# zoj613/OccuSpytial

Hardware: AMD Instinct MI355X
Metric: Gibbs iterations/sec on 100x100 ICAR lattice, 4 chains; 1/2/4/8 GPUs (higher is better)
Workload: dtype f64; 1 GPU; 100x100 queen ICAR lattice, 10000 sites, 5 visits/site, p=q=2, 4 chains per GPU batched in every kernel (BASELINE configs[1] data, the metric's 4 chains); chains_per_gpu=4, total_chains=4, sites=10000, visit_rows=50000, parallelism=chains sharded 4/GPU, no data-path collective; one GPU, communicator=single process, problem_transport=none, krylov_cap=0, stalls=0, solve_form=k_iter, one XCD per chain, solve_workgroups_per_chain=23, main_stream_cus=160, fused_fallbacks=0, threads_per_block=64

## Files before the change

### occuspytial_amd/csrc/occ_gibbs.hip

```cpp
#include "../../include/occ_gibbs.h"

#include <hip/hip_runtime.h>
#include <hip/hip_ext.h>

#include <algorithm>
#include <chrono>
#include <cmath>
#include <cstdio>
#include <cstdlib>
#include <cstring>
#include <atomic>
#include <map>
#include <mutex>
#include <string>
#include <thread>
#include <vector>

#include "occ_comm.hpp"
#include "occ_tiles.hpp"
#include "occ_comp.hpp"
#include "occ_rsr.hpp"
#include "occ_probit.hpp"
#include "occ_spatial.hpp"
#include "occ_hist.hpp"
// ... 109 lines not shown
        CompArgs args{};
        std::vector<void *> dev;
    } comp;
    bool comp_on() const { return comp.args.k > 1; }
    struct Switches {
        uint32_t any = 0u;
        std::vector<uint32_t> on;
        uint32_t *on_dev = nullptr;
    };
    struct Spatial : Switches {
        SpArgs args{};
    } spatial;
    struct AccumRun : Switches {
        bool ready = false, snapped = false;
        uint8_t *data = nullptr, *count = nullptr, *snap = nullptr;
        size_t unit = 0;
    };
    struct Hist : AccumRun {
        std::vector<uint64_t> bound;
        HistArgs args{};
    } hist;
    struct Conv : AccumRun {
        ConvArgs args{};
    } conv;
    struct Holdout : AccumRun {
        std::vector<double> packed;
        HoldoutArgs args{};
    } holdout;
    AccumRun &accum(int kind) { return kind == ACC_HIST ? (AccumRun &)hist : kind == ACC_CONV ? (AccumRun &)conv : (AccumRun &)holdout; }
    std::vector<ChainScalars> snap_sc;
    std::vector<std::pair<void *, size_t>> fixed_list;
    std::vector<const char *> fixed_names;
    bool defer_fixed = false;
    std::string group_transport = "none";
    Inject *inj_dev = nullptr;
    double *inj_u = nullptr;
    int snap_parity = 0;
    int64_t fused_fallbacks = 0;
    bool streams_serialised = false;
    unsigned *probe_w = nullptr;
    unsigned long long probe_gen = 0;
    int64_t stream_probes = 0, repromotions = 0;
    unsigned *sync_buf = nullptr;
    bool demoted = false;
    int promote_wait = 0, promote_backoff = 1;
    std::string pair_note;
    std::vector<ChainScalars> mirror;
    bool mirror_ok = false;
    bool clean_exit = false;
    ChainScalars *pin_sc = nullptr;
    double *pin_rec = nullptr;
    size_t pin_rec_cap = 0;
    bool marks_done = false;
    bool debug_close_window = false;
    bool wedged = false;
    int probe_wait = 0, probe_backoff = 1;
    int graph_parity = 0;
    std::vector<void *> allocs;
    std::string err;
    int launch_rc = 0;
    std::string launch_err;
    int parity = 0;
    bool need_prologue = true;
    hipGraph_t head_graph[2] = {nullptr, nullptr}, tail_graph[2] = {nullptr, nullptr};
    hipGraphExec_t head[2] = {nullptr, nullptr}, tail[2] = {nullptr, nullptr};
    hipEvent_t ev_z[2] = {nullptr, nullptr}, ev_side[2] = {nullptr, nullptr};
    int krylov_cap = 0;
    int64_t iterations = 0, graph_launches = 0, eager_iterations = 0, stalls = 0;
    int krylov_last = 0;
    double last_run_ms = 0.0;
    double profile_minres_iterations = 0.0;
    double profile_iter_dispatch_us = 0.0;
    hipEvent_t ext_ev0 = nullptr, ext_ev1 = nullptr;
    int calib_max = 0;
    unsigned long long seen_tot = 0, seen_sq = 0, seen_solves = 0;
    double *rec_buf = nullptr;
    size_t rec_cap = 0;
    std::vector<int32_t> site_id, site_ptr;
    std::vector<uint8_t> obs_site;
    bool probit = false;
    PbArgs pb{};
    std::vector<double> pb_K, pb_Phi, pb_G;
    hipGraph_t pb_graph = nullptr;
    hipGraphExec_t pb_exec = nullptr;
};

namespace {

#define HIP_TRY(expr)                                                                              \
    do {                                                                                           \
        hipError_t e_ = (expr);                                                                    \
        if (e_ != hipSuccess) {                                                                    \
            s->err = std::string(#expr) + ": " + hipGetErrorString(e_);                            \
            return OCC_E_HIP;                                                                      \
        }                                                                                          \
    } while (0)

static std::string host_state(const occ_sampler *s)
{
    char buf[512];
    std::snprintf(buf, sizeof(buf),
                  "device %d, %d chains, n %d; path: form %d (created %d) rsr_m %d; hand-overs: flag_sync %d side_enabled %d "
                  "event_nodes %d demoted %d streams_serialised %d; main_cus %d (%s pair); parity %d graph_parity %d snap_parity %d; "
                  "mirror_ok %d clean_exit %d need_prologue %d; graph launches %lld, eager iterations %lld, fallbacks %lld",
                  s->device, s->ctx.C, s->ctx.n, s->run.form, s->plan.form, s->rsr.m, (int)s->run.flag_sync, (int)s->plan.side_enabled,
                  (int)s->plan.event_nodes, (int)s->demoted, (int)s->streams_serialised, s->run.main_cus, (s->pair && !s->pair->m_main.empty()) ? "CU-masked" : "plain",
                  s->parity, s->graph_parity, s->snap_parity, (int)s->mirror_ok, (int)s->clean_exit, (int)s->need_prologue,
                  (long long)s->graph_launches, (long long)s->eager_iterations, (long long)s->fused_fallbacks);
    return buf;
}
static double host_wait_limit_s()
{
    const char *e = std::getenv("OCC_HOST_WAIT_S");
    const double v = e ? std::atof(e) : 20.0;
    return v > 0.0 ? v : 20.0;
}
static hipError_t poll_stream(hipStream_t st, bool *late)
{
    *late = false;
    const auto t0 = std::chrono::steady_clock::now();
    const double limit = host_wait_limit_s();
    for (unsigned polls = 1;; ++polls) {
        const hipError_t q = hipStreamQuery(st);
        if (q != hipErrorNotReady) return q;
        (void)hipGetLastError();
        if ((polls & 63u) == 0u) {
            const double sec = std::chrono::duration<double>(std::chrono::steady_clock::now() - t0).count();
            if (sec > limit) { *late = true; return hipErrorNotReady; }
            if (sec > 0.002) std::this_thread::yield();
        }
    }
}
static int wait_on(occ_sampler *s, hipStream_t st, const char *func, int line)
{
    const std::string what = std::string(func) + " (occ_gibbs.hip:" + std::to_string(line) + ")";
    if (!st) return OCC_OK;
    bool late = false;
    const hipError_t e = poll_stream(st, &late);
    if (e == hipSuccess) return OCC_OK;
    if (late) {
        s->wedged = true;
        if (s->pair) {
            std::lock_guard<std::mutex> g(g_pool_mu);
            s->pair->dead = true;
        }
        char lim[64];
        std::snprintf(lim, sizeof(lim), "%.0f s", host_wait_limit_s());
        s->err = std::string("host wait `") + what + "`: the " + (st == s->side ? "side" : "main") + " stream did not drain within " + lim +
                 " (every device-side wait of the engine is bounded far below that: the queue is not being served); " + host_state(s);
// ... 270 lines not shown
            for (int base = 0; base < (fm == FORM_XCD ? c.C : 1); base += XL_SLOTS) {
                IterArgs ia = s->iter;
                ia.chain_base = base;
                if (s->ext_ev0 && base == 0) hipExtLaunchKernelGGL(k, grid, bt, lds, st, s->ext_ev0, s->ext_ev1, 0, ia, e, fl);
                else hipLaunchKernelGGL(k, grid, bt, lds, st, ia, e, fl);
            }
            break;
        }
        default:
            if (P.tpb == 64) {
                const unsigned nb4 = (unsigned)((c.n + 255) / 256);
                if (P.generic) hipLaunchKernelGGL((k_beta_draw<0, 0>), dim3((unsigned)c.C), dim3(256), 0, st, OCC_ARGS);
                hipLaunchKernelGGL(z_ob, P.generic ? dim3(nb4 * 2, (unsigned)c.C) : shared_grid(c, 0, (int)nb4 * 2), dim3(256), 0, st, OCC_ARGS,
                                   (s->launch_sync ? 1 : 0) | 2 | P.zob_flags);
            } else {
                if (P.generic) hipLaunchKernelGGL((k_beta_draw<0, 0>), dim3((unsigned)c.C), dim3(256), 0, st, OCC_ARGS);
                else if (P.beta_split) hipLaunchKernelGGL(OCC_PICK_P(k_beta_draw, c.p), dim3((unsigned)c.C), dim3(64), 0, st, OCC_ARGS);
                hipLaunchKernelGGL(z_ob, dim3((unsigned)c.nb_n * 2, (unsigned)c.C), blk, 0, st, OCC_ARGS,
                                   (s->launch_sync ? 1 : 0) | P.zob_flags | (P.beta_split ? 4 : 0));
            }
            if (s->spatial.any)
                sp_launch(s->spatial.args, s->ctx.sc, c.C, e, st);
            if (s->hist.any)
                hist_launch(s->hist.args, s->ctx.sc, c.C, e, st);
            if (s->conv.any)
                conv_launch(s->conv.args, s->ctx.sc, c.C, e, st);
            if (s->holdout.any)
                holdout_launch(s->holdout.args, s->ctx.sc, c.C, e, st);
            break;
    }
    const hipError_t le = hipGetLastError();
    if (le != hipSuccess) {
        s->err = std::string("launch of ") + kind_name(kind) + " failed: " + hipGetErrorString(le);
        return OCC_E_HIP;
    }
    return OCC_OK;
}
#define LAUNCH(...)                                          \
    do {                                                     \
        const int lrc_ = launch_kind(__VA_ARGS__);           \
        if (lrc_ != OCC_OK && s->launch_rc == OCC_OK) {      \
            s->launch_rc = lrc_;                             \
            s->launch_err = s->err;                          \
        }                                                    \
    } while (0)
int take_launch_rc(occ_sampler *s)
{
    const int rc = s->launch_rc;
    if (rc != OCC_OK) s->err = s->launch_err;
    s->launch_rc = OCC_OK;
    return rc;
}

int read_scalars(occ_sampler *s, std::vector<ChainScalars> &h)
{
    h.resize(s->ctx.C);
    if (s->run.flag_sync) WAIT_TRY(s->side);
    if (!s->pin_sc) HIP_TRY(hipHostMalloc((void **)&s->pin_sc, 2 * sizeof(ChainScalars) * h.size(), hipHostMallocDefault));
    ChainScalars *back = s->pin_sc + h.size();
    HIP_TRY(hipMemcpyAsync(back, s->ctx.sc, sizeof(ChainScalars) * h.size(), hipMemcpyDeviceToHost, s->stream));
    WAIT_TRY(s->stream);
    std::memcpy(h.data(), back, sizeof(ChainScalars) * h.size());
    return OCC_OK;
}
int write_scalars(occ_sampler *s, const std::vector<ChainScalars> &h)
{
    s->mirror_ok = false;
    HIP_TRY(hipMemcpyAsync(s->ctx.sc, h.data(), sizeof(ChainScalars) * h.size(), hipMemcpyHostToDevice, s->stream));
    WAIT_TRY(s->stream);
    return OCC_OK;
}

int check_device_errors(occ_sampler *s, const std::vector<ChainScalars> &h)
{
    for (size_t c = 0; c < h.size(); ++c) {
        if (h[c].err == OCC_E_MINRES) { s->err = "MINRES solver did not converge!"; return OCC_E_MINRES; }
        if (h[c].err == OCC_E_CHOLESKY) { s->err = "Cholesky factorization/solver failed!"; return OCC_E_CHOLESKY; }
        if (h[c].err == OCC_E_HIP) {
            s->device_timeout = true;
            s->err = "a device-side wait timed out (a barrier among the workgroups of a chain in k_iter, or a hand-over "
                     "between the two streams): the device is over-subscribed or its queues are being serialised; "
                     "OCC_EVENT_SYNC=1 hands over through events, OCC_NO_PERSISTENT=1 uses one launch per MINRES step";
            return OCC_E_HIP;
        }
    }
    return OCC_OK;
}

int launch_prologue(occ_sampler *s)
{
    LAUNCH(s, s->stream, K_OMEGA_B, s->parity);
    LAUNCH(s, s->stream, K_NOISE, s->parity, 0);
    s->need_prologue = false;
    return take_launch_rc(s);
}

int eager_krylov(occ_sampler *s, int k_from, int *k_last)
{
    std::vector<Slot> slots((size_t)s->ctx.C * NSLOT);
    for (int k = k_from;; ++k) {
        LAUNCH(s, s->stream, K_MINRES, s->parity, k);
        if (k < 4) continue;
        HIP_TRY(hipMemcpyAsync(slots.data(), s->ctx.slots, sizeof(Slot) * slots.size(), hipMemcpyDeviceToHost, s->stream));
        WAIT_TRY(s->stream);
        if (int lrc = take_launch_rc(s)) return lrc;
        bool all = true;
        for (int c = 0; c < s->ctx.C; ++c) all = all && slots[(size_t)c * NSLOT + (k & (NSLOT - 1))].done;
        if (all) {
            *k_last = k;
            return OCC_OK;
        }
        if ((long long)k > s->ctx.maxiter + 3) return set_error(s, OCC_E_MINRES, "MINRES solver did not converge!");
    }
}
// ... 46 lines not shown
        s->tail_graph[e] = nullptr;
    }
}

int graph_leaf(occ_sampler *s, hipGraph_t graph, hipGraphNode_t *leaf)
{
    size_t n = 0;
    HIP_TRY(hipGraphGetNodes(graph, nullptr, &n));
    std::vector<hipGraphNode_t> nodes(n);
    HIP_TRY(hipGraphGetNodes(graph, nodes.data(), &n));
    for (hipGraphNode_t nd : nodes) {
        size_t deps = 0;
        HIP_TRY(hipGraphNodeGetDependentNodes(nd, nullptr, &deps));
        if (deps == 0) { *leaf = nd; return OCC_OK; }
    }
    return set_error(s, OCC_E_HIP, "captured graph has no leaf node");
}

int capture_graph(occ_sampler *s, hipStream_t st, SeqWhere where, int p, int n_seq, int cap, hipEvent_t wait_ev, hipEvent_t rec_ev, hipGraph_t *graph)
{
    const SeqMode mode = seq_mode(s);
    const SeqParts parts = seq_parts(mode, where);
    const SeqGate gate = seq_gate(mode, std::getenv("OCC_GATE_KERNEL") != nullptr);
    bool open = false;
    hipGraphNode_t node = nullptr;
    auto end_capture = [&]() -> int {
        hipGraph_t g = nullptr;
        if (open) HIP_TRY(hipStreamEndCapture(st, &g));
        if (open && !*graph) *graph = g;
        open = false;
        return OCC_OK;
    };
    int rc;
    for (int t = 0; t < n_seq; ++t)
        for (int i = 0; i < parts.n; ++i) {
            const SeqPart part = parts.part[i];
            if (part == PART_WAIT || part == PART_RECORD) {
                hipGraphNode_t leaf = nullptr;
                if ((rc = end_capture())) return rc;
                if (!*graph) HIP_TRY(hipGraphCreate(graph, 0));
                else if ((rc = graph_leaf(s, *graph, &leaf))) return rc;
                if (part == PART_WAIT) HIP_TRY(hipGraphAddEventWaitNode(&node, *graph, leaf ? &leaf : nullptr, leaf ? 1 : 0, wait_ev));
                else HIP_TRY(hipGraphAddEventRecordNode(&node, *graph, leaf ? &leaf : nullptr, leaf ? 1 : 0, rec_ev));
                continue;
            }
            if (!open && *graph) HIP_TRY(hipStreamBeginCaptureToGraph(st, *graph, &node, nullptr, 1, hipStreamCaptureModeThreadLocal));
            else if (!open) HIP_TRY(hipStreamBeginCapture(st, hipStreamCaptureModeThreadLocal));
            open = true;
            walk(s, st, SeqParts{1, {part}}, seq_solve(s, false), seq_parity(p, t), cap, gate);
        }
    return end_capture();
}

int build_graph(occ_sampler *s, int cap)
{
    const auto host_t0 = std::chrono::steady_clock::now();
    WAIT_TRY(s->stream);
    destroy_head(s);
    const SeqMode mode = seq_mode(s);
    if (!seq_mode_runs(mode, seq_solve(s, false)))
        return set_error(s, OCC_E_HIP, "hand-overs by device counters need a solve of one launch or the reduced-rank model: no graph to capture");
    const int n_seq = sequences_per_enqueue(mode);
    Scoped<bool> sync(&s->launch_sync, mode == SEQ_RSR_ONE_STREAM ? false : s->launch_sync);
    if (mode == SEQ_COUNTERS) {
        WAIT_TRY(s->side);
        HIP_TRY(fill_on(s, s->ctx.sync, 0, sizeof(unsigned) * SYNC_DEBUG));
    }
    int rc;
    for (int g = 0; g < (n_seq > 1 ? 1 : 2); ++g) {
        const int p = n_seq > 1 ? s->parity : g;
        if ((rc = capture_graph(s, s->stream, ON_MAIN, p, n_seq, cap, s->ev_side[p], s->ev_z[p], &s->head_graph[g]))) return rc;
        HIP_TRY(hipGraphInstantiate(&s->head[g], s->head_graph[g], nullptr, nullptr, 0));
        if (s->tail[g] || seq_parts(mode, ON_SIDE).n == 0) continue;
        if ((rc = capture_graph(s, s->side, ON_SIDE, p, n_seq, cap, s->ev_z[p ^ 1], s->ev_side[p], &s->tail_graph[g]))) return rc;
        HIP_TRY(hipGraphInstantiate(&s->tail[g], s->tail_graph[g], nullptr, nullptr, 0));
    }
    if (n_seq > 1) s->graph_parity = s->parity;
    s->krylov_cap = cap;
    if (std::getenv("OCC_VERBOSE")) {
        const double ms = std::chrono::duration<double, std::milli>(std::chrono::steady_clock::now() - host_t0).count();
        std::fprintf(stderr, "[occ] graphs captured, Krylov cap %d: %.2f ms host time\n", cap, ms);
    }
    return take_launch_rc(s);
}

int enqueue_sequence(occ_sampler *s)
{
    const int e = s->parity;
    const SeqMode mode = seq_mode(s);
    switch (mode) {
        case SEQ_COUNTERS:
            HIP_TRY(hipGraphLaunch(s->tail[0], s->side));
            [[fallthrough]];
        case SEQ_RSR_ONE_STREAM:
            HIP_TRY(hipGraphLaunch(s->head[0], s->stream));
            return OCC_OK;
        case SEQ_EVENT_NODES:
            HIP_TRY(hipGraphLaunch(s->tail[e], s->side));
            HIP_TRY(hipGraphLaunch(s->head[e], s->stream));
            break;
        case SEQ_STREAM_EVENTS:
            HIP_TRY(hipStreamWaitEvent(s->side, s->ev_z[e ^ 1], 0));
            HIP_TRY(hipGraphLaunch(s->tail[e], s->side));
            HIP_TRY(hipEventRecord(s->ev_side[e], s->side));
            HIP_TRY(hipGraphLaunch(s->head[e], s->stream));
            HIP_TRY(hipStreamWaitEvent(s->stream, s->ev_side[e], 0));
            break;
        case SEQ_ONE_STREAM:
            HIP_TRY(hipGraphLaunch(s->tail[e], s->stream));
            HIP_TRY(hipGraphLaunch(s->head[e], s->stream));
            break;
    }
    walk(s, s->stream, seq_parts(mode, BEHIND), seq_solve(s, false), e);
    if (mode == SEQ_STREAM_EVENTS) HIP_TRY(hipEventRecord(s->ev_z[e], s->stream));
    s->parity ^= 1;
    return take_launch_rc(s);
}

int get_scalars(occ_sampler *s, std::vector<ChainScalars> &h)
{
    if (s->mirror_ok) { h = s->mirror; return OCC_OK; }
    return read_scalars(s, h);
}

int open_window(occ_sampler *s, int64_t n_iter, int64_t burnin, int64_t keep, bool snapshot, bool run)
{
    const Ctx &c = s->ctx;
    std::vector<ChainScalars> h;
    int rc = get_scalars(s, h);
    if (rc) return rc;
    s->mirror_ok = false;
    if (!s->clean_exit) {
        if (c.claim) HIP_TRY(hipMemsetAsync(c.claim, 0, sizeof(unsigned) * (size_t)c.C * 16, s->stream));
        if (c.sync) HIP_TRY(hipMemsetAsync(c.sync + SYNC_ABORT, 0, sizeof(unsigned), s->stream));
    }
    s->clean_exit = false;
    const uint32_t dev_n = s->debug_close_window ? 0u : (uint32_t)n_iter;
    s->debug_close_window = false;
    if (snapshot) {
        const size_t Cn = (size_t)c.C * c.n;
        if (!s->snap_eta) {
            if ((rc = dev_alloc(s, &s->snap_eta, Cn, false))) return rc;
            if ((rc = dev_alloc(s, &s->snap_z, Cn, false))) return rc;
            if ((rc = dev_alloc(s, &s->snap_x, Cn, false))) return rc;
            if (s->rsr.m > 0 && (rc = dev_alloc(s, &s->snap_theta, (size_t)c.C * s->rsr.m, false))) return rc;
        }
        s->snap_sc = h;
        s->snap_parity = s->parity;
// ... 1575 lines not shown
    DeviceLease lease = lease_device(s->device);
    HIP_TRY(hipSetDevice(s->device));
    if (s->probit) {
        std::vector<PbChain> hp;
        int rc = pb_read_chains(s, hp);
        if (rc) return rc;
        for (size_t c = 0; c < hp.size(); ++c) hp[c].key = keys[c];
        return pb_write_chains(s, hp);
    }
    std::vector<ChainScalars> h;
    int rc = read_scalars(s, h);
    if (rc) return rc;
    for (size_t c = 0; c < h.size(); ++c) h[c].key = keys[c];
    s->need_prologue = true;
    return write_scalars(s, h);
}

static int step_impl(occ_sampler *s, bool snapshot)
{
    int rc = open_window(s, 1, 0, 0, snapshot, false);
    if (rc) return rc;
    if ((rc = eager_sequence(s))) return rc;
    std::vector<ChainScalars> h;
    if ((rc = read_scalars(s, h))) return rc;
    s->iterations = h[0].ctl[s->parity].it;
    s->krylov_last = h[0].minres_itn_last;
    if ((rc = check_device_errors(s, h))) return rc;
    s->mirror = h;
    s->mirror_ok = true;
    s->clean_exit = true;
    return OCC_OK;
}

static int finish_marks(occ_sampler *s, bool last, size_t n_rec)
{
    if (!last) return OCC_OK;
    HIP_TRY(hipEventRecord(s->ev1, s->stream));
    const int grc = grow_pinned(s, &s->pin_rec, &s->pin_rec_cap, n_rec);
    if (grc) return grc;
    if (n_rec) HIP_TRY(hipMemcpyAsync(s->pin_rec, s->rec_buf, sizeof(double) * n_rec, hipMemcpyDeviceToHost, s->stream));
    const int rrc = records_copy_out(s);
    if (rrc) return rrc;
    s->marks_done = true;
    return OCC_OK;
}

static int run_impl(occ_sampler *s, int64_t n_iter, int64_t burnin, double *out_alpha, double *out_beta, double *out_tau, bool snapshot)
{
    Ctx &c = s->ctx;
    const int C = c.C, p = c.p, q = c.q;
    const int64_t keep = n_iter - burnin;
    const size_t rw = (size_t)q + p + 1;
    const size_t need = (size_t)C * keep * rw;
    int rc = grow_device(s, &s->rec_buf, &s->rec_cap, need);
    if (rc) return rc;
    if ((rc = records_open(s, C, keep))) return rc;
    if ((rc = records_publish(s))) return rc;
    if ((rc = open_window(s, n_iter, burnin, keep, snapshot, true))) return rc;
    std::vector<ChainScalars> h;
    HIP_TRY(hipEventRecord(s->ev0, s->stream));
    s->marks_done = false;

    const SeqMode mode = seq_mode(s);
    const SeqSolve solve = seq_solve(s, false);
    const int64_t seq_per_enqueue = sequences_per_enqueue(mode);
    int64_t done_min = 0;
    const char *force = std::getenv("OCC_FORCE_KRYLOV_CAP");
    if (std::getenv("OCC_EAGER_ONLY")) {
        for (int64_t i = 0; i < n_iter; ++i)
            if ((rc = eager_sequence(s))) return rc;
        done_min = n_iter;
    } else if (solve == SOLVE_FUSED && seq_per_enqueue == 1) {
        if (!s->head[0] && (rc = build_graph(s, 0))) return rc;
        if (s->need_prologue && (rc = launch_prologue(s))) return rc;
    } else if (seq_per_enqueue > 1) {
        if (s->need_prologue && (rc = launch_prologue(s))) return rc;
        if (s->head[0] && s->parity != s->graph_parity) {
            if ((rc = eager_sequence(s))) return rc;
            done_min = 1;
        }
        if (!s->head[0] && n_iter > 1 && (rc = build_graph(s, 0))) return rc;
        if (n_iter == 1 && done_min == 0) {
            if ((rc = eager_sequence(s))) return rc;
            done_min = 1;
        }
    } else if (!s->head[0]) {
        const int64_t n_calib = std::min<int64_t>(n_iter, 3);
        s->calib_max = 0;
        for (int64_t i = 0; i < n_calib; ++i) {
            if (i == n_calib - 1) s->calib_max = 0;
            if ((rc = eager_sequence(s))) return rc;
        }
        done_min = n_calib;
        int cap = std::max(4, s->calib_max + 2);
        if (force) cap = std::max(1, std::atoi(force));
        if (done_min < n_iter && (rc = build_graph(s, cap))) return rc;
    } else if (s->need_prologue) {
        if ((rc = launch_prologue(s))) return rc;
    }
    if (done_min < n_iter && (mode == SEQ_EVENT_NODES || mode == SEQ_STREAM_EVENTS)) HIP_TRY(hipEventRecord(s->ev_z[s->parity ^ 1], s->stream));

    std::vector<std::pair<uint32_t, uint32_t>> seen((size_t)C, {0xffffffffu, 0xffffffffu});
    while (done_min < n_iter) {
        const int64_t left = n_iter - done_min;
        int64_t batch = std::min<int64_t>(left, s->graph_launches < 128 ? 32 : 256);
        batch = (batch + seq_per_enqueue - 1) / seq_per_enqueue * seq_per_enqueue;
        const auto hl0 = std::chrono::steady_clock::now();
        for (int64_t b = 0; b < batch; b += seq_per_enqueue)
            if ((rc = enqueue_sequence(s))) return rc;
        const auto hl1 = std::chrono::steady_clock::now();
        s->graph_launches += batch;
        if ((rc = finish_marks(s, done_min + batch >= n_iter, (size_t)C * keep * rw))) return rc;
        if ((rc = read_scalars(s, h))) return rc;
        if (std::getenv("OCC_VERBOSE")) {
            const auto hl2 = std::chrono::steady_clock::now();
            std::fprintf(stderr, "[occ] host: %.1f us per sequence to enqueue, %.1f us per sequence until the batch finished\n",
                         std::chrono::duration<double, std::micro>(hl1 - hl0).count() / batch,
                         std::chrono::duration<double, std::micro>(hl2 - hl0).count() / batch);
        }
        if ((rc = check_device_errors(s, h))) return rc;
        done_min = n_iter;
        unsigned long long tot = 0, sq = 0, solves = 0;
        for (int ch = 0; ch < C; ++ch) {
            done_min = std::min<int64_t>(done_min, (int64_t)h[ch].ctl[s->parity].it - (int64_t)h[ch].it_base);
            tot += h[ch].krylov_total; sq += h[ch].krylov_sq_total; solves += h[ch].solves;
        }
        for (int ch = 0; ch < C; ++ch) {
            const Ctl &ctl = h[ch].ctl[s->parity];
            const bool unfinished = (int64_t)ctl.it - (int64_t)h[ch].it_base < n_iter;
            if (unfinished && seen[(size_t)ch].first == ctl.it && seen[(size_t)ch].second == ctl.koff) {
                std::string msg = "no progress: a batch of " + std::to_string((long long)batch) + " sequences left chain " + std::to_string(ch) +
                                  " where it was (the window of iterations is not open on the device?); per chain {it, koff | other parity | mid | it_base, it_stop, err}:";
                for (int k2 = 0; k2 < C && k2 < 16; ++k2) {
                    const ChainScalars &q2 = h[k2];
                    char b[192];
                    std::snprintf(b, sizeof(b), " [%d] {%u, %u | %u, %u | %u, %u / %u, %u | %u, %u, %d}", k2, q2.ctl[s->parity].it, q2.ctl[s->parity].koff, q2.ctl[s->parity ^ 1].it,
                                  q2.ctl[s->parity ^ 1].koff, q2.mid[0].it, q2.mid[0].koff, q2.mid[1].it, q2.mid[1].koff, q2.it_base, q2.it_stop, (int)q2.err);
                    msg += b;
                }
                msg += "; the host wanted " + std::to_string((long long)n_iter) + " iterations, done_min " + std::to_string((long long)done_min) + "; " + host_state(s);
                return set_error(s, OCC_E_HIP, msg.c_str());
            }
            seen[(size_t)ch] = {ctl.it, ctl.koff};
        }
        if (std::getenv("OCC_VERBOSE")) {
            unsigned long long car = 0;
            for (int ch = 0; ch < C; ++ch) car += h[ch].carries;
            std::fprintf(stderr, "[occ] batch of %lld sequences: done_min %lld / %lld, carries so far %llu, cap %d\n",
                         (long long)batch, (long long)done_min, (long long)n_iter, car, s->krylov_cap);
        }
        const unsigned long long ds = solves - s->seen_solves;
        if (!force && solve == SOLVE_CAPTURED && ds >= 32 && done_min < n_iter) {
            const double mean = (double)(tot - s->seen_tot) / ds;
            const double var = std::max(0.0, (double)(sq - s->seen_sq) / ds - mean * mean);
            const int want = std::max(4, (int)std::ceil(mean + 2.5 * std::sqrt(var)));
            s->seen_tot = tot; s->seen_sq = sq; s->seen_solves = solves;
            if ((want > s->krylov_cap || want < s->krylov_cap - 1) && (rc = build_graph(s, want))) return rc;
        }
    }
    if (!s->marks_done) {
        if ((rc = finish_marks(s, true, (size_t)C * keep * rw))) return rc;
        if ((rc = read_scalars(s, h))) return rc;
        if ((rc = check_device_errors(s, h))) return rc;
    }
    float ms = 0.f;
    HIP_TRY(hipEventElapsedTime(&ms, s->ev0, s->ev1));
    s->last_run_ms = ms;
    s->iterations = h[0].ctl[s->parity].it;
    s->krylov_last = h[0].minres_itn_last;
    s->mirror = h;
    s->mirror_ok = true;
    s->clean_exit = true;

    split_rows(s->pin_rec, C, keep, q, p, out_alpha, out_beta, out_tau);
    records_close(s, keep, h);
    return OCC_OK;
}


static int set_handover(occ_sampler *s, bool flags)
{
    if (s->run.flag_sync == flags) return OCC_OK;
    WAIT_TRY(s->stream);
    WAIT_TRY(s->side);
    destroy_graph(s);
    s->run.flag_sync = flags;
    s->ctx.sync = flags ? s->sync_buf : nullptr;
    s->iter.sync = s->ctx.sync;
    s->rsr.sync = s->ctx.sync;
    if (flags) HIP_TRY(fill_on(s, s->sync_buf, 0, sizeof(unsigned) * SYNC_WORDS));
    HIP_TRY(copy_on(s, s->ctx_dev, &s->ctx, sizeof(Ctx), hipMemcpyHostToDevice));
    return OCC_OK;
}

static int fallback_to_launch_per_step(occ_sampler *s)
{
    Ctx &c = s->ctx;
    const size_t Cn = (size_t)c.C * c.n;
    WAIT_TRY(s->stream);
    WAIT_TRY(s->side);
    (void)hipGetLastError();
    if (std::getenv("OCC_VERBOSE") || !std::getenv("OCC_QUIET"))
        std::fprintf(stderr, "[occ] %s -- re-running the call without hand-overs between the streams%s\n",
                     s->err.c_str(), s->rsr.m > 0 ? "" : ", one launch per MINRES step");
    destroy_graph(s);
    s->device_timeout = false;
    s->launch_rc = OCC_OK;
    int rc;
    if ((rc = drop_to_launch_per_step(s))) return rc;
    HIP_TRY(copy_on(s, c.eta, s->snap_eta, sizeof(double) * Cn, hipMemcpyDeviceToDevice));
    HIP_TRY(copy_on(s, c.z, s->snap_z, Cn, hipMemcpyDeviceToDevice));
    HIP_TRY(copy_on(s, c.Xv, s->snap_x, sizeof(double2) * Cn, hipMemcpyDeviceToDevice));
    if (s->rsr.m > 0) HIP_TRY(copy_on(s, s->rsr.theta, s->snap_theta, sizeof(double) * (size_t)c.C * s->rsr.m, hipMemcpyDeviceToDevice));
    for (int k = 0; k < N_SUMS; ++k) {
        const size_t nsum = (size_t)SUMS[k].nacc * Cn;
        if (!s->sums[k].snapped) continue;
        HIP_TRY(copy_on(s, c.*SUMS[k].acc, s->sums[k].snap, sizeof(double) * nsum, hipMemcpyDeviceToDevice));
        HIP_TRY(copy_on(s, c.*SUMS[k].count, s->sums[k].snap + nsum, sizeof(double) * (size_t)c.C, hipMemcpyDeviceToDevice));
    }
    for (int k = 0; k < N_ACCUM; ++k) {
        const occ_sampler::AccumRun &r = s->accum(k);
        const size_t nd = (size_t)ACCUM[k].elem * accum_words(ACCUM[k], (size_t)c.C, r.unit);
        if (!r.snapped) continue;
        HIP_TRY(copy_on(s, r.data, r.snap, nd, hipMemcpyDeviceToDevice));
        HIP_TRY(copy_on(s, r.count, r.snap + nd, (size_t)ACCUM[k].elem * (size_t)c.C, hipMemcpyDeviceToDevice));
    }
    for (auto &sc : s->snap_sc) sc.err = 0;
    if ((rc = write_scalars(s, s->snap_sc))) return rc;
    s->parity = s->snap_parity;
// ... 55 lines not shown
    bool ask = s->probe_gen != g_stream_gen.load();
    if (!ask && s->streams_serialised && !s->run.flag_sync && --s->probe_wait <= 0) ask = true;
    if (!s->demoted && s->run.main_cus > 0 && s->sync_buf && s->plan.flag_sync && ask) {
        bool beside = true;
        if ((rc = stream_probe(s, &beside))) return rc;
        s->streams_serialised = !beside;
        if (beside) s->probe_backoff = 1;
        else { s->probe_backoff = std::min(64, s->probe_backoff * 2); s->probe_wait = s->probe_backoff; }
        if ((rc = set_handover(s, beside))) return rc;
    }
    return OCC_OK;
}

static int hist_admit(occ_sampler *s, int64_t add)
{
    occ_sampler::Hist &hs = s->hist;
    if (!hs.any) return OCC_OK;
    for (size_t ch = 0; ch < hs.on.size(); ++ch)
        if (hs.on[ch] && hs.bound[ch] + (uint64_t)add > 0xffffffffull)
            return set_error(s, OCC_E_BADARG, ("this call could take a count of the per-site histograms of chain " + std::to_string(ch) +
                                               " past 2^32 - 1: read hist_counts and set hist_stats again first").c_str());
    for (size_t ch = 0; ch < hs.on.size(); ++ch)
        if (hs.on[ch]) hs.bound[ch] += (uint64_t)add;
    return OCC_OK;
}

int occ_step(occ_sampler *s)
{
    if (!s) return OCC_E_BADARG;
    DeviceLease lease = lease_device(s->device);
    HIP_TRY(hipSetDevice(s->device));
    if (s->probit) return pb_step(s);
    int rc;
    if ((rc = hist_admit(s, 1))) return rc;
    if ((rc = refresh_paths(s))) return rc;
    const bool fused = (s->fused() && s->rsr.m == 0) || s->run.flag_sync;
    s->device_timeout = false;
    rc = step_impl(s, fused);
    if (rc == OCC_E_HIP && fused && s->device_timeout) {
        if ((rc = fallback_to_launch_per_step(s))) return rc;
        rc = step_impl(s, false);
    }
    return rc;
}

int occ_run(occ_sampler *s, int64_t n_iter, int64_t burnin, double *out_alpha, double *out_beta, double *out_tau)
{
    if (!s) return OCC_E_BADARG;
    if (n_iter < 1 || burnin < 0 || burnin >= n_iter) return set_error(s, OCC_E_BADARG, "burnin value cannot be larger than sample size");
    if (!out_alpha || !out_beta || !out_tau) return set_error(s, OCC_E_BADARG, "null output buffer");
    DeviceLease lease = lease_device(s->device);
    HIP_TRY(hipSetDevice(s->device));
    if (s->probit) return pb_run(s, n_iter, burnin, out_alpha, out_beta, out_tau);
    int rc;
    if ((rc = hist_admit(s, n_iter - burnin))) return rc;
    if ((rc = refresh_paths(s))) return rc;
    const bool fused = (s->fused() && s->rsr.m == 0) || s->run.flag_sync;
    s->device_timeout = false;
    rc = run_impl(s, n_iter, burnin, out_alpha, out_beta, out_tau, fused);
    if (rc == OCC_E_HIP && fused && s->device_timeout) {
        if ((rc = fallback_to_launch_per_step(s))) return rc;
        rc = run_impl(s, n_iter, burnin, out_alpha, out_beta, out_tau, false);
    }
    return rc;
}

enum : int { SITE_NONE = -1, SITE_COUNT = -2, SITE_SWITCH = -3 };
static int site_field(const std::string &nm, int *kind)
{
    for (int k = 0; k < N_SUMS; ++k) {
        *kind = k;
        if (nm == SUMS[k].sw) return SITE_SWITCH;
        if (nm == SUMS[k].cnt) return SITE_COUNT;
        for (int q = 0; q < SUMS[k].nacc; ++q)
            if (nm == SUMS[k].sum[q]) return q;
    }
    return SITE_NONE;
}
static int sums_refused(occ_sampler *s, const SumsKind &k)
{
    return set_error(s, OCC_E_STATE, (std::string(k.what) + " are not available for the probit model").c_str());
}

static int flip_output(occ_sampler *s, std::vector<ChainScalars> &h, int chain, uint32_t bit, bool on)
{
    const int level_before = s->z_ob_kind();
    s->outputs_on = 0u;
    if (s->probit) {
        std::vector<uint32_t> &pb_on = s->regions.pb_on;
        pb_on[(size_t)chain] = on;
        HIP_TRY(copy_on(s, s->regions.pb_on_dev, pb_on.data(), sizeof(uint32_t) * pb_on.size(), hipMemcpyHostToDevice));
        for (uint32_t o : pb_on) s->outputs_on |= o ? bit : 0u;
    } else {
        h[(size_t)chain].site_on = (h[(size_t)chain].site_on & ~bit) | (on ? bit : 0u);
        const int rc = write_scalars(s, h);
        if (rc) return rc;
        for (const ChainScalars &sc : h) s->outputs_on |= sc.site_on;
    }
    if (s->z_ob_kind() == level_before) return OCC_OK;
    if (!s->probit) {
        destroy_graph(s);
        return OCC_OK;
    }
    if (s->pb_exec) (void)hipGraphExecDestroy(s->pb_exec);
    if (s->pb_graph) (void)hipGraphDestroy(s->pb_graph);
    s->pb_exec = nullptr;
    s->pb_graph = nullptr;
    return OCC_OK;
}

static int set_site_state(occ_sampler *s, int chain, int kind, int field, const double *in, int64_t len)
{
    const SumsKind &k = SUMS[kind];
    if (s->probit) return sums_refused(s, k);
    Ctx &c = s->ctx;
    const size_t n = (size_t)c.n, Cn = (size_t)c.C * n;
// ... 1097 lines not shown
```

### occuspytial_amd/csrc/occ_plan.hpp

```cpp
#pragma once
#include "../../include/occ_gibbs.h"

#include <algorithm>
#include <climits>
#include <cmath>
#include <cstdint>
#include <string>
#include <vector>

namespace occ {

constexpr int MAXC = 8;
constexpr int NPRE = 8;
constexpr int nacc(int d) { return d * (d + 1) / 2 + d; }
constexpr int ITER_WG = 256;
constexpr int ITER_WG_XL = 512;
constexpr int ITER_SITES_SW = 448;
constexpr int XL_MAX_WG = 64;
constexpr int XL_SLOTS = 8;
constexpr int TILE = 256;
constexpr int tiles_wg_per_cu(int T) { return T == 1 ? 4 : (T == 4 ? 2 : 3); }
constexpr int RSR_MAX_DIM = 128;
constexpr int TILES_GB_DEFAULT = 1;

// ... 149 lines not shown
}

inline void plan_granted(Plan &P, bool granted)
{
    const PlanOptions &o = P.opt;
    const int n = P.shape.n, C = P.shape.chains;
    granted = granted && P.partition;
    P.main_cus = granted ? P.nmain : 0;
    P.share_on = granted ? P.share_on : 0;
    const int cus = P.main_cus > 0 ? P.main_cus : P.ncu;
    P.any_fits = P.any && (long long)P.nbg * C <= (long long)(P.iter_window == 8 ? 2 : 1) * cus;
    const bool trust = o.skip_residency_probe;
    const int hot_cus = P.main_cus > 0 ? P.main_hot_cus : P.ncu / XL_SLOTS;
    if (!trust && P.xl && P.xl_nbg > P.xl_per_cu * hot_cus) P.xl = false;
    if (P.tiles && !trust && (long long)P.tiles_G * C > (long long)tiles_wg_per_cu(P.tiles_T) * cus) P.tiles = false;
    P.persistent = P.xl || P.any_fits || P.tiles;
    if (!P.persistent) P.tpb = P.tpb_plain;
    if (!P.persistent && P.shape.rsr_dim == 0) P.main_cus = P.share_on = 0;
    const int tpb = P.tpb, nb_n = P.nb_n = (n + tpb - 1) / tpb;
    P.beta_split = tpb != 64 && nb_n >= 128 && !o.no_beta_split;
    P.nb_r = std::max(1, (P.shape.rows + tpb - 1) / tpb);
    if (P.share_on) {
        const int per_chain[3] = {tpb == 64 ? 2 * ((n + 255) / 256) : 2 * P.nb_n, P.nb_r, (n + 255) / 256}, which[3] = {0, 1, 1};
        P.surplus_last = o.surplus_last;
        if (o.main_share != KNOB_UNSET) {
            const int w = o.main_share, hot = std::min(C, XL_SLOTS);
            for (int x = hot; x < XL_SLOTS; ++x) P.share_cum[0][x + 1] = P.share_cum[0][x] + w;
        }
        for (int k = 0; k < 3; ++k) {
            const long long T = (long long)per_chain[k] * C, W = P.share_cum[which[k]][8];
            for (int x = 0; x <= XL_SLOTS; ++x) P.tile_first[k][x] = (int)(T * P.share_cum[which[k]][x] / W);
            for (int x = 0; x < XL_SLOTS; ++x) P.tile_most[k] = std::max(P.tile_most[k], P.tile_first[k][x + 1] - P.tile_first[k][x]);
        }
    }
    if (P.tiles) P.ladder.push_back({FORM_TILES, P.nbg, 0});
    if (P.xl) P.ladder.push_back({FORM_XCD, P.xl_nbg, P.xl_wide});
    if (P.any_fits) P.ladder.push_back({FORM_ANY, P.nbg, 0});
    P.ladder.push_back({FORM_STEPS, P.nbg, 0});
}

inline void plan_settle(Plan &P, int form)
{
    P.form = form;
    if (form == FORM_STEPS && P.persistent) P.main_cus = P.share_on = 0;
    P.flag_sync = P.main_cus > 0 && !P.opt.event_sync;
}

enum Kind { K_OMEGA_B = 0, K_NOISE, K_ETA_INIT, K_MINRES, K_BETA_PARTIAL, K_OMEGA_A, K_ALPHA_DRAW, K_Z_OB, K_ITER, K_GATE ,
            K_RSR_GRAM, K_RSR_SOLVE, K_RSR_ETA_BETA ,
            K_COMP_PART, K_COMP_COEF, K_COMP_ETA, K_COMP_BETA  };
static_assert(K_ITER + 1 == OCC_N_KERNEL_KINDS, "kernel kinds out of sync with the header");

constexpr int GRAPH_SEQ = 2;

enum SeqMode : int {
    SEQ_COUNTERS = 0,
    SEQ_RSR_ONE_STREAM = 1,
    SEQ_EVENT_NODES = 2,
    SEQ_STREAM_EVENTS = 3,
    SEQ_ONE_STREAM = 4
};
constexpr SeqMode seq_mode(bool flag_sync, bool rsr, bool event_nodes, bool side_enabled)
{
    return flag_sync ? SEQ_COUNTERS : rsr ? SEQ_RSR_ONE_STREAM : event_nodes ? SEQ_EVENT_NODES : side_enabled ? SEQ_STREAM_EVENTS : SEQ_ONE_STREAM;
}
constexpr int sequences_per_enqueue(SeqMode m) { return m <= SEQ_RSR_ONE_STREAM ? GRAPH_SEQ : 1; }
constexpr int seq_parity(int p, int t) { return p ^ (t & 1); }

enum SeqSolve : int { SOLVE_RSR = 0, SOLVE_FUSED, SOLVE_CAPTURED, SOLVE_EAGER };
constexpr bool seq_mode_runs(SeqMode m, SeqSolve sv) { return m == SEQ_COUNTERS ? sv <= SOLVE_FUSED : m != SEQ_RSR_ONE_STREAM || sv == SOLVE_RSR; }
enum SeqGate : int { GATE_NONE = 0, GATE_IN_OMEGA_A, GATE_KERNEL };
constexpr SeqGate seq_gate(SeqMode m, bool as_kernel) { return m != SEQ_COUNTERS ? GATE_NONE : as_kernel ? GATE_KERNEL : GATE_IN_OMEGA_A; }

enum SeqPart : int { PART_SIDE = 0, PART_SOLVE, PART_TAIL, PART_WAIT , PART_RECORD  };
struct SeqLaunch { int kind, e, extra; };
constexpr int EXTRA_HOST_WATCHED = -1, EXTRA_K_LAST = -2;

template <class Emit>
void seq_launches(SeqPart part, SeqSolve sv, int e, int cap, SeqGate gate, Emit &&emit, bool comp = false)
{
    auto correction = [&]() {
        if (comp)
            for (int k : {K_COMP_PART, K_COMP_COEF, K_COMP_ETA, K_COMP_BETA}) emit(SeqLaunch{k, e, 0});
    };
    switch (part) {
        case PART_SIDE:
            if (gate == GATE_KERNEL) emit(SeqLaunch{K_GATE, 0, 0});
            emit(SeqLaunch{K_OMEGA_A, e, gate == GATE_IN_OMEGA_A ? 1 : 0});
            emit(SeqLaunch{K_NOISE, e, 1});
            break;
        case PART_SOLVE:
            if (sv == SOLVE_RSR)
                for (int k : {K_RSR_GRAM, K_RSR_SOLVE, K_RSR_ETA_BETA}) emit(SeqLaunch{k, e, 0});
            if (sv == SOLVE_FUSED) {
                emit(SeqLaunch{K_ITER, e, 0});
                correction();
            }
            if (sv <= SOLVE_FUSED) break;
            emit(SeqLaunch{K_ETA_INIT, e, 0});
            if (sv == SOLVE_EAGER) emit(SeqLaunch{K_MINRES, e, EXTRA_HOST_WATCHED});
            else for (int k = 1; k <= cap + 3; ++k) emit(SeqLaunch{K_MINRES, e, k});
            emit(SeqLaunch{K_BETA_PARTIAL, e, sv == SOLVE_EAGER ? EXTRA_K_LAST : cap + 3});
            correction();
            break;
        case PART_TAIL: emit(SeqLaunch{K_Z_OB, e, 0}); break;
        default: break;
    }
}

enum SeqWhere : int { ON_MAIN = 0, ON_SIDE, BEHIND };
struct SeqParts { int n; SeqPart part[4]; };
constexpr SeqParts seq_parts(SeqMode m, SeqWhere w)
{
    switch (m) {
        case SEQ_COUNTERS: return w == ON_MAIN ? SeqParts{2, {PART_SOLVE, PART_TAIL}} : w == ON_SIDE ? SeqParts{1, {PART_SIDE}} : SeqParts{0, {}};
        case SEQ_RSR_ONE_STREAM: return w == ON_MAIN ? SeqParts{3, {PART_SIDE, PART_SOLVE, PART_TAIL}} : SeqParts{0, {}};
        case SEQ_EVENT_NODES:
            return w == ON_MAIN ? SeqParts{4, {PART_SOLVE, PART_WAIT, PART_TAIL, PART_RECORD}} : w == ON_SIDE ? SeqParts{3, {PART_WAIT, PART_SIDE, PART_RECORD}} : SeqParts{0, {}};
        default: return w == ON_MAIN ? SeqParts{1, {PART_SOLVE}} : w == ON_SIDE ? SeqParts{1, {PART_SIDE}} : SeqParts{1, {PART_TAIL}};
    }
}
constexpr SeqParts seq_eager() { return SeqParts{3, {PART_SIDE, PART_SOLVE, PART_TAIL}}; }

constexpr uint32_t OUT_SITE = 1u, OUT_LL = 2u, OUT_REGION = 4u, OUT_PPC = 8u;
struct Output { uint32_t bit; int level; const char *sw; bool probit; };
constexpr int N_OUTPUTS = 4;
constexpr Output OUTPUTS[N_OUTPUTS] = {{OUT_SITE, 1, "site_stats", false},
                                       {OUT_LL, 2, "ll_stats", false},
                                       {OUT_REGION, 3, "region_stats", true},
                                       {OUT_PPC, 4, "ppc_stats", false}};
constexpr const Output &output_of(uint32_t bit) { return OUTPUTS[bit == OUT_SITE ? 0 : bit == OUT_LL ? 1 : bit == OUT_REGION ? 2 : 3]; }
static_assert(output_of(OUT_SITE).bit == OUT_SITE && output_of(OUT_LL).bit == OUT_LL && output_of(OUT_REGION).bit == OUT_REGION && output_of(OUT_PPC).bit == OUT_PPC, "output_of");
constexpr int output_level(uint32_t on)
{
    int level = 0;
    for (int k = 0; k < N_OUTPUTS; ++k)
        if ((on & OUTPUTS[k].bit) && OUTPUTS[k].level > level) level = OUTPUTS[k].level;
    return level;
}

}
```

### occuspytial_amd/csrc/occ_plan_capi.cpp

```cpp
#include <cstdio>
#include <cstring>

#include "occ_accum.hpp"
#include "occ_draws.hpp"
#include "occ_layout.hpp"

using namespace occ;

extern "C" {

struct OccPlanOut {
    int32_t form, main_cus, tpb, nb_n, nb_r, beta_split, share_on, surplus_last, iter_window, generic, nbg;
    int32_t tiles_T, tiles_G, xl_wide, xl_nbg, xl_per_cu, main_hot_cus, nmain, partition, flag_sync;
    int32_t per_xcd[XL_SLOTS], tile_first[3][XL_SLOTS + 1], tile_most[3];
    int32_t n_ladder, ladder_form[4], ladder_nbg[4];
};

int occ_plan_eval(const int32_t shape[8], int32_t ncu, const PlanOptions *opt, int32_t granted, OccPlanOut *out, char *err, int32_t errlen)
{
    PlanShape sh;
    sh.n = shape[0]; sh.rows = shape[1]; sh.chains = shape[2]; sh.p = shape[3]; sh.q = shape[4];
    sh.rsr_dim = shape[5]; sh.wmax = shape[6]; sh.dia = shape[7] != 0;
    Plan P;
    std::string why;
    if (!plan_wanted(sh, ncu, *opt, &P, &why)) {
        std::snprintf(err, (size_t)errlen, "%s", why.c_str());
        return -1;
    }
    plan_granted(P, granted != 0);
    plan_settle(P, P.ladder.front().form);
    *out = OccPlanOut{};
    out->form = P.form; out->main_cus = P.main_cus; out->tpb = P.tpb; out->nb_n = P.nb_n; out->nb_r = P.nb_r;
    out->beta_split = P.beta_split; out->share_on = P.share_on; out->surplus_last = P.surplus_last;
    out->iter_window = P.iter_window; out->generic = P.generic; out->nbg = P.nbg;
    out->tiles_T = P.tiles_T; out->tiles_G = P.tiles_G; out->xl_wide = P.xl_wide; out->xl_nbg = P.xl_nbg;
    out->xl_per_cu = P.xl_per_cu; out->main_hot_cus = P.main_hot_cus; out->nmain = P.nmain; out->partition = P.partition;
    out->flag_sync = P.flag_sync;
    for (int x = 0; x < XL_SLOTS; ++x) out->per_xcd[x] = P.per_xcd[x];
    for (int k = 0; k < 3; ++k) {
        for (int x = 0; x <= XL_SLOTS; ++x) out->tile_first[k][x] = P.tile_first[k][x];
        out->tile_most[k] = P.tile_most[k];
    }
    out->n_ladder = (int32_t)P.ladder.size();
    for (size_t i = 0; i < P.ladder.size() && i < 4; ++i) { out->ladder_form[i] = P.ladder[i].form; out->ladder_nbg[i] = P.ladder[i].nbg; }
    return 0;
}

int32_t occ_order_mode(int32_t flag_sync, int32_t rsr, int32_t event_nodes, int32_t side_enabled, int32_t solve)
{
    const SeqMode m = seq_mode(flag_sync != 0, rsr != 0, event_nodes != 0, side_enabled != 0);
    return seq_mode_runs(m, (SeqSolve)solve) ? (int32_t)m : -1;
}
int32_t occ_order_sequences_per_enqueue(int32_t mode) { return sequences_per_enqueue((SeqMode)mode); }

int32_t occ_order_launches_comp(int32_t mode, int32_t where, int32_t solve, int32_t p, int32_t cap, int32_t gate_kernel, int32_t comp, int32_t *out, int32_t max);
int32_t occ_order_launches(int32_t mode, int32_t where, int32_t solve, int32_t p, int32_t cap, int32_t gate_kernel, int32_t *out, int32_t max)
{
    return occ_order_launches_comp(mode, where, solve, p, cap, gate_kernel, 0, out, max);
}
int32_t occ_order_launches_comp(int32_t mode, int32_t where, int32_t solve, int32_t p, int32_t cap, int32_t gate_kernel, int32_t comp, int32_t *out, int32_t max)
{
    const SeqMode m = (SeqMode)mode;
    const SeqParts parts = where == 3 ? seq_eager() : seq_parts(m, (SeqWhere)where);
    int32_t n = 0;
    for (int t = 0; t < (where == 3 ? 1 : sequences_per_enqueue(m)); ++t)
        for (int i = 0; i < parts.n; ++i) {
            auto emit = [&](const SeqLaunch &l) {
                if (n < max) { out[3 * n] = l.kind; out[3 * n + 1] = l.e; out[3 * n + 2] = l.extra; }
                ++n;
            };
            if (parts.part[i] == PART_WAIT || parts.part[i] == PART_RECORD) emit(SeqLaunch{parts.part[i] == PART_WAIT ? -1 : -2, seq_parity(p, t), 0});
            else seq_launches(parts.part[i], (SeqSolve)solve, seq_parity(p, t), cap, where == 3 ? GATE_NONE : seq_gate(m, gate_kernel != 0), emit, comp != 0);
        }
    return n <= max ? n : -1;
}

int32_t occ_output_count(void) { return N_OUTPUTS; }
uint32_t occ_output_row(int32_t k, int32_t *level, const char **sw, int32_t *probit)
{
    *level = OUTPUTS[k].level; *sw = OUTPUTS[k].sw; *probit = OUTPUTS[k].probit;
    return OUTPUTS[k].bit;
}
int32_t occ_output_level(uint32_t on) { return output_level(on); }

int32_t occ_accum_count(void) { return N_ACCUM; }
void occ_accum_row(int32_t k, const char **what, const char *name[4], const char *refusal[4], int32_t num[3], double range[2])
{
    const Accum &a = ACCUM[k];
    *what = a.what;
    for (int f = 0; f < 4; ++f) name[f] = a.name[f];
    refusal[0] = a.not_ready; refusal[1] = a.bad_switch; refusal[2] = a.bad_count; refusal[3] = a.bad_data;
    num[0] = a.elem; num[1] = a.slots; num[2] = a.cnt_slot;
    range[0] = a.on_min; range[1] = a.on_max;
}
int64_t occ_accum_words(int32_t k, int64_t C, int64_t unit) { return (int64_t)accum_words(ACCUM[k], (size_t)C, (size_t)unit); }
int64_t occ_accum_offset(int64_t C, int64_t unit, int64_t slot, int64_t chain) { return (int64_t)accum_offset((size_t)C, (size_t)unit, (size_t)slot, (size_t)chain); }
int32_t occ_accum_lookup(const char *name, int32_t *field) { return accum_lookup(name, field); }
int32_t occ_accum_switch_ok(int32_t k, double v) { return accum_switch_ok(ACCUM[k], v); }
const char *occ_accum_write_refusal(int32_t k, int32_t field, const double *in, int64_t len, int64_t unit)
{
    return accum_write_refusal(ACCUM[k], field, in, (size_t)len, (size_t)unit);
}

int32_t occ_draws_count(void) { return N_DRAWS; }
void occ_draws_row(int32_t k, const char *name[3], const char *refusal[5], int32_t num[6])
{
// ... 73 lines not shown
```

Before: 78690 iterations/s.

## Capture longer graph sequences, launch main before side, join streams on device

Adds an eight-sequence graph variant that is used whenever at least eight iterations remain in a batch. This cuts the number of hipGraphLaunch calls per batch. In counters mode the main graph is now launched before the side graph, and read_scalars joins the side stream through an event instead of blocking the host on it. It also sets a minimum size for the record buffer and adds optional timestamps printed under OCC_VERBOSE, at the cost of extra graph instantiation and memory.

```diff
diff --git a/occuspytial_amd/csrc/occ_gibbs.hip b/occuspytial_amd/csrc/occ_gibbs.hip
--- a/occuspytial_amd/csrc/occ_gibbs.hip
+++ b/occuspytial_amd/csrc/occ_gibbs.hip
@@ -185,6 +185,8 @@
     double *pin_rec = nullptr;
     size_t pin_rec_cap = 0;
     bool marks_done = false;
+    bool stamps_on = false;
+    std::vector<std::pair<const char *, std::chrono::steady_clock::time_point>> stamps;
     bool debug_close_window = false;
     bool wedged = false;
     int probe_wait = 0, probe_backoff = 1;
@@ -228,6 +230,11 @@
             return OCC_E_HIP;                                                                      \
         }                                                                                          \
     } while (0)
+
+static inline void stamp(occ_sampler *s, const char *stage)
+{
+    if (s->stamps_on) s->stamps.emplace_back(stage, std::chrono::steady_clock::now());
+}
 
 static std::string host_state(const occ_sampler *s)
 {
@@ -604,14 +611,23 @@
     return rc;
 }
 
-int read_scalars(occ_sampler *s, std::vector<ChainScalars> &h)
+int read_scalars(occ_sampler *s, std::vector<ChainScalars> &h, bool join_on_device = false)
 {
     h.resize(s->ctx.C);
-    if (s->run.flag_sync) WAIT_TRY(s->side);
+    if (s->run.flag_sync && join_on_device) {
+        HIP_TRY(hipEventRecord(s->ev_side[0], s->side));
+        HIP_TRY(hipStreamWaitEvent(s->stream, s->ev_side[0], 0));
+    } else if (s->run.flag_sync) {
+        WAIT_TRY(s->side);
+    }
+    stamp(s, "read_scalars: side stream joined");
     if (!s->pin_sc) HIP_TRY(hipHostMalloc((void **)&s->pin_sc, 2 * sizeof(ChainScalars) * h.size(), hipHostMallocDefault));
     ChainScalars *back = s->pin_sc + h.size();
     HIP_TRY(hipMemcpyAsync(back, s->ctx.sc, sizeof(ChainScalars) * h.size(), hipMemcpyDeviceToHost, s->stream));
+    stamp(s, "read_scalars: copy enqueued");
     WAIT_TRY(s->stream);
+    if (s->run.flag_sync && join_on_device) WAIT_TRY(s->side);
+    stamp(s, "read_scalars: main stream drained");
     std::memcpy(h.data(), back, sizeof(ChainScalars) * h.size());
     return OCC_OK;
 }
@@ -764,7 +780,7 @@
     return end_capture();
 }
 
-int build_graph(occ_sampler *s, int cap)
+int build_graph(occ_sampler *s, int cap, bool with_long = false)
 {
     const auto host_t0 = std::chrono::steady_clock::now();
     WAIT_TRY(s->stream);
@@ -779,12 +795,13 @@
         HIP_TRY(fill_on(s, s->ctx.sync, 0, sizeof(unsigned) * SYNC_DEBUG));
     }
     int rc;
-    for (int g = 0; g < (n_seq > 1 ? 1 : 2); ++g) {
+    for (int g = 0; g < (n_seq > 1 && !with_long ? 1 : 2); ++g) {
         const int p = n_seq > 1 ? s->parity : g;
-        if ((rc = capture_graph(s, s->stream, ON_MAIN, p, n_seq, cap, s->ev_side[p], s->ev_z[p], &s->head_graph[g]))) return rc;
+        const int len = n_seq > 1 && g == 1 ? GRAPH_SEQ_LONG : n_seq;
+        if ((rc = capture_graph(s, s->stream, ON_MAIN, p, len, cap, s->ev_side[p], s->ev_z[p], &s->head_graph[g]))) return rc;
         HIP_TRY(hipGraphInstantiate(&s->head[g], s->head_graph[g], nullptr, nullptr, 0));
         if (s->tail[g] || seq_parts(mode, ON_SIDE).n == 0) continue;
-        if ((rc = capture_graph(s, s->side, ON_SIDE, p, n_seq, cap, s->ev_z[p ^ 1], s->ev_side[p], &s->tail_graph[g]))) return rc;
+        if ((rc = capture_graph(s, s->side, ON_SIDE, p, len, cap, s->ev_z[p ^ 1], s->ev_side[p], &s->tail_graph[g]))) return rc;
         HIP_TRY(hipGraphInstantiate(&s->tail[g], s->tail_graph[g], nullptr, nullptr, 0));
     }
     if (n_seq > 1) s->graph_parity = s->parity;
@@ -796,16 +813,21 @@
     return take_launch_rc(s);
 }
 
-int enqueue_sequence(occ_sampler *s)
+int enqueue_sequence(occ_sampler *s, int len = GRAPH_SEQ)
 {
     const int e = s->parity;
     const SeqMode mode = seq_mode(s);
+    const int g = len == GRAPH_SEQ_LONG ? 1 : 0;
+    static_assert(seq_main_first(SEQ_COUNTERS) && !seq_main_first(SEQ_EVENT_NODES) && !seq_main_first(SEQ_STREAM_EVENTS) && !seq_main_first(SEQ_ONE_STREAM),
+                  "the order of each mode's two launches below is occ_plan.hpp's");
     switch (mode) {
         case SEQ_COUNTERS:
-            HIP_TRY(hipGraphLaunch(s->tail[0], s->side));
-            [[fallthrough]];
+            HIP_TRY(hipGraphLaunch(s->head[g], s->stream));
+            stamp(s, "main graph launched");
+            HIP_TRY(hipGraphLaunch(s->tail[g], s->side));
+            return OCC_OK;
         case SEQ_RSR_ONE_STREAM:
-            HIP_TRY(hipGraphLaunch(s->head[0], s->stream));
+            HIP_TRY(hipGraphLaunch(s->head[g], s->stream));
             return OCC_OK;
         case SEQ_EVENT_NODES:
             HIP_TRY(hipGraphLaunch(s->tail[e], s->side));
@@ -2487,13 +2509,20 @@
     const int64_t keep = n_iter - burnin;
     const size_t rw = (size_t)q + p + 1;
     const size_t need = (size_t)C * keep * rw;
-    int rc = grow_device(s, &s->rec_buf, &s->rec_cap, need);
+    stamp(s, "run_impl entered");
+    constexpr size_t REC_FLOOR = 8192;
+    int rc = grow_device(s, &s->rec_buf, &s->rec_cap, std::max(need, REC_FLOOR));
     if (rc) return rc;
+    stamp(s, "rec_buf grown");
     if ((rc = records_open(s, C, keep))) return rc;
+    stamp(s, "records_open");
     if ((rc = records_publish(s))) return rc;
+    stamp(s, "records_publish");
     if ((rc = open_window(s, n_iter, burnin, keep, snapshot, true))) return rc;
+    stamp(s, "open_window");
     std::vector<ChainScalars> h;
     HIP_TRY(hipEventRecord(s->ev0, s->stream));
+    stamp(s, "ev0");
     s->marks_done = false;
 
     const SeqMode mode = seq_mode(s);
@@ -2514,7 +2543,7 @@
             if ((rc = eager_sequence(s))) return rc;
             done_min = 1;
         }
-        if (!s->head[0] && n_iter > 1 && (rc = build_graph(s, 0))) return rc;
+        if (!s->head[0] && n_iter > 1 && (rc = build_graph(s, 0, true))) return rc;
         if (n_iter == 1 && done_min == 0) {
             if ((rc = eager_sequence(s))) return rc;
             done_min = 1;
@@ -2541,12 +2570,18 @@
         int64_t batch = std::min<int64_t>(left, s->graph_launches < 128 ? 32 : 256);
         batch = (batch + seq_per_enqueue - 1) / seq_per_enqueue * seq_per_enqueue;
         const auto hl0 = std::chrono::steady_clock::now();
-        for (int64_t b = 0; b < batch; b += seq_per_enqueue)
-            if ((rc = enqueue_sequence(s))) return rc;
+        stamp(s, "first enqueue reached");
+        for (int64_t b = 0; b < batch;) {
+            const int len = seq_per_enqueue > 1 ? graph_len(batch - b, s->head[1] != nullptr) : 1;
+            if ((rc = enqueue_sequence(s, len))) return rc;
+            stamp(s, "enqueue_sequence");
+            b += len;
+        }
         const auto hl1 = std::chrono::steady_clock::now();
         s->graph_launches += batch;
         if ((rc = finish_marks(s, done_min + batch >= n_iter, (size_t)C * keep * rw))) return rc;
-        if ((rc = read_scalars(s, h))) return rc;
+        stamp(s, "finish_marks");
+        if ((rc = read_scalars(s, h, true))) return rc;
         if (std::getenv("OCC_VERBOSE")) {
             const auto hl2 = std::chrono::steady_clock::now();
             std::fprintf(stderr, "[occ] host: %.1f us per sequence to enqueue, %.1f us per sequence until the batch finished\n",
@@ -2595,7 +2630,7 @@
     }
     if (!s->marks_done) {
         if ((rc = finish_marks(s, true, (size_t)C * keep * rw))) return rc;
-        if ((rc = read_scalars(s, h))) return rc;
+        if ((rc = read_scalars(s, h, true))) return rc;
         if ((rc = check_device_errors(s, h))) return rc;
     }
     float ms = 0.f;
@@ -2609,7 +2644,16 @@
 
     split_rows(s->pin_rec, C, keep, q, p, out_alpha, out_beta, out_tau);
     records_close(s, keep, h);
-    return OCC_OK;
+    stamp(s, "rows split, records closed");
+    return OCC_OK;
+}
+
+static void print_stamps(occ_sampler *s)
+{
+    for (size_t i = 1; i < s->stamps.size(); ++i)
+        std::fprintf(stderr, "[occ] stamp %9.1f us  +%8.1f  %s\n", std::chrono::duration<double, std::micro>(s->stamps[i].second - s->stamps[0].second).count(),
+                     std::chrono::duration<double, std::micro>(s->stamps[i].second - s->stamps[i - 1].second).count(), s->stamps[i].first);
+    s->stamps.clear();
 }
 
 
@@ -2771,6 +2815,9 @@
     DeviceLease lease = lease_device(s->device);
     HIP_TRY(hipSetDevice(s->device));
     if (s->probit) return pb_run(s, n_iter, burnin, out_alpha, out_beta, out_tau);
+    Scoped<bool> stamps(&s->stamps_on, std::getenv("OCC_VERBOSE") != nullptr);
+    s->stamps.clear();
+    stamp(s, "occ_run entered");
     int rc;
     if ((rc = hist_admit(s, n_iter - burnin))) return rc;
     if ((rc = refresh_paths(s))) return rc;
@@ -2781,6 +2828,7 @@
         if ((rc = fallback_to_launch_per_step(s))) return rc;
         rc = run_impl(s, n_iter, burnin, out_alpha, out_beta, out_tau, false);
     }
+    print_stamps(s);
     return rc;
 }
 
diff --git a/occuspytial_amd/csrc/occ_plan.hpp b/occuspytial_amd/csrc/occ_plan.hpp
--- a/occuspytial_amd/csrc/occ_plan.hpp
+++ b/occuspytial_amd/csrc/occ_plan.hpp
@@ -225,6 +225,8 @@
 static_assert(K_ITER + 1 == OCC_N_KERNEL_KINDS, "kernel kinds out of sync with the header");
 
 constexpr int GRAPH_SEQ = 2;
+constexpr int GRAPH_SEQ_LONG = 8;
+constexpr int graph_len(long long left, bool have_long) { return have_long && left >= GRAPH_SEQ_LONG ? GRAPH_SEQ_LONG : GRAPH_SEQ; }
 
 enum SeqMode : int {
     SEQ_COUNTERS = 0,
@@ -293,6 +295,7 @@
         default: return w == ON_MAIN ? SeqParts{1, {PART_SOLVE}} : w == ON_SIDE ? SeqParts{1, {PART_SIDE}} : SeqParts{1, {PART_TAIL}};
     }
 }
+constexpr bool seq_main_first(SeqMode m) { return m == SEQ_COUNTERS; }
 constexpr SeqParts seq_eager() { return SeqParts{3, {PART_SIDE, PART_SOLVE, PART_TAIL}}; }
 
 constexpr uint32_t OUT_SITE = 1u, OUT_LL = 2u, OUT_REGION = 4u, OUT_PPC = 8u;
diff --git a/occuspytial_amd/csrc/occ_plan_capi.cpp b/occuspytial_amd/csrc/occ_plan_capi.cpp
--- a/occuspytial_amd/csrc/occ_plan_capi.cpp
+++ b/occuspytial_amd/csrc/occ_plan_capi.cpp
@@ -52,6 +52,9 @@
     return seq_mode_runs(m, (SeqSolve)solve) ? (int32_t)m : -1;
 }
 int32_t occ_order_sequences_per_enqueue(int32_t mode) { return sequences_per_enqueue((SeqMode)mode); }
+int32_t occ_order_graph_seq_long(void) { return GRAPH_SEQ_LONG; }
+int32_t occ_order_graph_len(int64_t left, int32_t have_long) { return graph_len(left, have_long != 0); }
+int32_t occ_order_main_first(int32_t mode) { return seq_main_first((SeqMode)mode); }
 
 int32_t occ_order_launches_comp(int32_t mode, int32_t where, int32_t solve, int32_t p, int32_t cap, int32_t gate_kernel, int32_t comp, int32_t *out, int32_t max);
 int32_t occ_order_launches(int32_t mode, int32_t where, int32_t solve, int32_t p, int32_t cap, int32_t gate_kernel, int32_t *out, int32_t max)
```

Result: faster. 83130 iterations/s, median of 6 (+5.6%).
